# FurkanOM/tf-ssd

Measured on AMD Instinct MI355X. Metric: images/sec SSD300 (MobileNetV2) fwd+NMS, higher is better.
Workload: dtype f32

## Files before the change

include/ssd_hip.h:

```cpp
#ifndef SSD_HIP_H
#define SSD_HIP_H

#include <stddef.h>
#include <stdint.h>

#ifdef __cplusplus
extern "C" {
#endif

#define SSD_OK 0
#define SSD_E_INVALID (-1)
#define SSD_E_HIP (-2)
#define SSD_E_UNSUPPORTED (-3)
#define SSD_E_STATE (-4)

const char* ssd_version(void);
const char* ssd_last_error(void);
int ssd_init(int device);
void* ssd_stream_create(int high_priority);
void* ssd_stream_create_masked(const unsigned* cu_mask, int words);
int ssd_stream_destroy(void* stream);

int ssd_priors_count(const int* fmaps, const int* n_ars, int levels);
int ssd_priors(const int* fmaps, const float* const* ars, const int* n_ars, int levels,
// ... 337 lines not shown
#define SSD_LOC_HUBER 0
#define SSD_LOC_IOU 1
#define SSD_LOC_GIOU 2
#define SSD_LOC_DIOU 3
#define SSD_LOC_CIOU 4
int ssd_iou_loc_loss_tile(void);
size_t ssd_iou_loc_loss_workspace_bytes(int B, int N);
int ssd_iou_loc_loss(const float* priors_dev, const float* variances, const float* actual_deltas_dev,
                     const float* pred_deltas_dev, int B, int N, int mode, float loc_loss_alpha,
                     float* loc_loss_dev, float* per_anchor_out_dev, float* grad_deltas_dev, float grad_scale,
                     void* workspace_dev, size_t workspace_bytes, void* stream);

#define SSD_LOSS_HARD_NEGATIVE 0
#define SSD_LOSS_FOCAL 1
typedef struct ssd_loss_config {
    int kind;
    float neg_pos_ratio, loc_loss_alpha, focal_alpha, focal_gamma;
    int loc_kind;
    const float* priors_dev;
    float variances[4];
} ssd_loss_config;
size_t ssd_loss_config_bytes(void);


enum ssd_act { SSD_ACT_NONE = 0, SSD_ACT_RELU = 1, SSD_ACT_RELU6 = 2 };

typedef struct ssd_conv_desc {
    int B, H, W, Cin;
    int Cout, kh, kw;
    int stride, dilation;
    int pad_t, pad_l, pad_b, pad_r;
    int act;
    int has_residual;
} ssd_conv_desc;

int ssd_same_pads(int in, int k, int stride, int dilation, int* before, int* after);
int ssd_conv_out_size(int in, int k, int stride, int dilation, int pad_before, int pad_after);

size_t ssd_conv_packed_weight_floats(int kh, int kw, int Cin, int Cout);
int ssd_conv_pack_weights(const float* hwio_dev, int kh, int kw, int Cin, int Cout,
                          float* packed_dev, void* stream);

int ssd_conv2d(const ssd_conv_desc* d, const float* in_dev, const float* packed_w_dev,
               const float* scale_dev, const float* shift_dev, const float* residual_dev,
               float* out_dev, long out_batch_stride, long out_pixel_stride, void* stream);

int ssd_conv_num_configs(void);
const char* ssd_conv_config_name(int config);
int ssd_conv2d_ex(const ssd_conv_desc* d, const float* in_dev, const float* packed_w_dev,
                  const float* scale_dev, const float* shift_dev, const float* residual_dev,
                  float* out_dev, long out_batch_stride, long out_pixel_stride, int config,
                  int split_k, float* splitk_ws_dev, void* stream);

int ssd_split_planes(const float* x_dev, long n, int channels, int planes, void* planes_dev, long plane_stride, void* stream);
int ssd_join_planes(const void* planes_dev, long n, int channels, int planes, long plane_stride, float* x_dev, void* stream);
int ssd_conv2d_planes(const ssd_conv_desc* d, const void* in_planes_dev, int planes, long in_plane_stride,
                      const float* packed_w_dev, const float* scale_dev, const float* shift_dev,
                      const float* residual_dev, float* out_dev, long out_batch_stride, long out_pixel_stride,
                      void* out_planes_dev, long out_plane_stride, int config, int split_k,
                      float* splitk_ws_dev, void* stream);

size_t ssd_conv_f16x2_weight_bytes(int kh, int kw, int Cin, int Cout);
int ssd_conv_pack_weights_f16x2(const float* packed_w_dev, int kh, int kw, int Cin, int Cout, void* w_planes_dev,
                                int* k_out, void* stream);
int ssd_conv2d_planes_f16x2(const ssd_conv_desc* d, const void* in_planes_dev, long in_plane_stride,
                            const float* packed_w_dev, const void* w_planes_dev, int w_exp, const float* scale_dev,
// ... 139 lines not shown
```

tf-ssd_amd/csrc/ssd_conv.h:

```cpp
#pragma once
#include <cmath>
#include <cstring>

#include "common.h"

namespace ssd {

struct ConvParams {
    const float* in;
    const float* w;
    const short* w3;
    const float* scale;
    const float* shift;
    const float* residual;
    float* out;
    int B, H, W, Cin, Ho, Wo, Cout;
    int kh, kw, stride, dil, pad_t, pad_l;
    int K, Kpad, Npad;
    long M;
    long out_batch_stride, out_pixel_stride;
    int n_split;
    float* out2;
    long out2_batch_stride, out2_pixel_stride;
    int vec_store2;
    int act;
    int vec_store;
    int split_k;
    float* partial;
    const float* wino_w;
    int bf16;
    const short* xp;
    long xp_plane;
    int xp_np;
    short* op;
    long op_plane;
    int op_np;
    const short* wh;
    float acc_scale;
};
inline int conv_vec_store(const ConvParams& p) {
    return (((uintptr_t)p.out & 15) == 0) && (p.out_pixel_stride % 4 == 0) && (p.out_batch_stride % 4 == 0);
}

struct FusedBlockParams {
    const float* x;
    float* y;
    const float* we;
    const float *es, *eh;
    const float* wd;
    const float *ds, *dh;
    const float* wp;
    const float *ps, *ph;
    int residual;
    int B, H, W, Cin, Ce, Cout, Ho, Wo, stride, pad_t, pad_l;
    int kpad_e, kpad_p, npad_p;
    int tiles_y, tiles_x;
    int bf16;
    int groups;
    const short* we3;
    const short* wp3;
    int bands;
    float* slabs;
    unsigned* tickets;
    float* e_out;
    short* y_planes;
    long y_plane;
    short* e_planes;
    long e_plane;
    int planes_np;
    int e_planes_np;
    int planes_only;
// ... 168 lines not shown
```

tf-ssd_amd/csrc/ssd_conv.hip:

```cpp
#include <cstring>

#include "ssd_conv.h"
#include "ssd_conv_mfma.h"

namespace ssd {


template <int V>
__global__ void splitk_reduce_kernel(const ConvParams p) {
    const long total = p.M * p.Cout;
    const long groups = total / V;
    const int HoWo = p.Ho * p.Wo;
    for (long g = (long)blockIdx.x * blockDim.x + threadIdx.x; g < groups; g += (long)gridDim.x * blockDim.x) {
        float t[V];
#pragma unroll
        for (int j = 0; j < V; ++j) t[j] = 0.f;
        for (int s = 0; s < p.split_k; ++s) {
            const float* src = p.partial + (long)s * total + g * V;
            if (V == 4) {
                const f32x4 v = *reinterpret_cast<const f32x4*>(src);
#pragma unroll
                for (int j = 0; j < V; ++j) t[j] += v[j];
            } else {
                t[0] += src[0];
// ... 400 lines not shown
    return SSD_OK;
}

int launch_pack_weights(const float* hwio, int K, int Cout, int Kpad, int Npad, float* packed, hipStream_t st) {
    const long total = (long)Npad * Kpad;
    if (total == 0) return SSD_OK;
    const int blocks = (int)(cdiv(total, 256) < 4096 ? cdiv(total, 256) : 4096);
    hipLaunchKernelGGL(pack_weights_kernel, dim3(blocks), dim3(256), 0, st, hwio, K, Cout, Kpad, Npad, packed);
    SSD_LAUNCH_CHECK();
    return SSD_OK;
}

int fill_conv_params(const ssd_conv_desc* d, ConvParams* p) {
    SSD_CHECK_ARG(d != nullptr, "conv2d: descriptor is NULL");
    SSD_CHECK_ARG(d->B >= 0 && d->H >= 1 && d->W >= 1 && d->Cin >= 1 && d->Cout >= 1,
                  "conv2d: bad tensor sizes B=%d H=%d W=%d Cin=%d Cout=%d", d->B, d->H, d->W, d->Cin, d->Cout);
    SSD_CHECK_ARG(d->kh >= 1 && d->kw >= 1 && d->stride >= 1 && d->dilation >= 1,
                  "conv2d: bad kernel %dx%d stride %d dilation %d", d->kh, d->kw, d->stride, d->dilation);
    SSD_CHECK_ARG(d->pad_t >= 0 && d->pad_l >= 0 && d->pad_b >= 0 && d->pad_r >= 0, "conv2d: negative padding");
    SSD_CHECK_ARG(d->act >= 0 && d->act <= 2, "conv2d: unknown activation %d", d->act);
    const int Ho = ssd_conv_out_size(d->H, d->kh, d->stride, d->dilation, d->pad_t, d->pad_b);
    const int Wo = ssd_conv_out_size(d->W, d->kw, d->stride, d->dilation, d->pad_l, d->pad_r);
    SSD_CHECK_ARG(Ho >= 1 && Wo >= 1, "conv2d: empty output (%d x %d)", Ho, Wo);
    *p = ConvParams{};
    p->B = d->B; p->H = d->H; p->W = d->W; p->Cin = d->Cin; p->Ho = Ho; p->Wo = Wo; p->Cout = d->Cout;
    p->kh = d->kh; p->kw = d->kw; p->stride = d->stride; p->dil = d->dilation;
    p->pad_t = d->pad_t; p->pad_l = d->pad_l;
    p->K = d->kh * d->kw * d->Cin;
    p->Kpad = conv_kpad(p->K);
    p->Npad = conv_npad(d->Cout);
    p->M = (long)d->B * Ho * Wo;
    p->act = d->act;
    p->split_k = 1;
    return SSD_OK;
}

}

using namespace ssd;

static int bind_conv_io(ConvParams& p, const ssd_conv_desc* d, const char* who, const float* residual_dev, float* out_dev,
                        long out_batch_stride, long out_pixel_stride, int split_k, float* splitk_ws_dev) {
    SSD_CHECK_ARG(!d->has_residual || residual_dev, "%s: has_residual set but residual is NULL", who);
    p.residual = d->has_residual ? residual_dev : nullptr;
    p.out = out_dev;
    p.out_pixel_stride = out_pixel_stride > 0 ? out_pixel_stride : p.Cout;
    p.out_batch_stride = out_batch_stride > 0 ? out_batch_stride : (long)p.Ho * p.Wo * p.out_pixel_stride;
    p.vec_store = conv_vec_store(p);
    if (split_k > 1) {
        SSD_CHECK_ARG(splitk_ws_dev != nullptr, "%s: split_k > 1 needs a workspace", who);
        p.split_k = split_k;
        p.partial = splitk_ws_dev;
    }
    return SSD_OK;
}

extern "C" {

int ssd_same_pads(int in, int k, int stride, int dilation, int* before, int* after) {
    if (in < 1 || k < 1 || stride < 1 || dilation < 1) return SSD_E_INVALID;
    const int out = (in + stride - 1) / stride;
    const int keff = (k - 1) * dilation + 1;
    int p = (out - 1) * stride + keff - in;
    if (p < 0) p = 0;
    if (before) *before = p / 2;
    if (after) *after = p - p / 2;
// ... 186 lines not shown
```

tf-ssd_amd/csrc/ssd_convdma.hip:

```cpp
#include "ssd_block_common.h"
#include "ssd_conv_mfma.h"

namespace ssd {

template <int MT, int NT, int WM, int WN, int NP, bool GEMM1X1, int KSH = 1>
__device__ __forceinline__ void conv_dma_body(const ConvParams& p, char* __restrict__ dsm) {
    constexpr int KS = NP == 1 ? 2 : NP == 2 ? KSH : 1;
    constexpr int WPL = NP == 1 ? 3 : 0;
    constexpr int BM = 16 * MT * WM, BN = 16 * NT * WN, NW = WM * WN;
    constexpr int RBX = BM / 16, RBW = BN / 16;
    constexpr int RPX = (RBX + NW - 1) / NW, RPW = (RBW + NW - 1) / NW;
    constexpr int XBYTES = KS * NP * BM * 64, STAGE = KS * NP * (BM + BN) * 64;

    const int tid = threadIdx.x, lane = tid & 63;
    const int wave = __builtin_amdgcn_readfirstlane(tid >> 6);
    const int wm = wave / WN, wn = wave % WN;
    const int nb_n = (p.Cout + BN - 1) / BN;
    const int mblk = blockIdx.x / nb_n, nblk = blockIdx.x - mblk * nb_n;
    const long m0 = (long)mblk * BM;
    const int n0 = nblk * BN;
    const int HoWo = p.Ho * p.Wo;
    const int ntaps = p.kh * p.kw;

    const int r16 = lane >> 2;
    const int q8 = ((lane & 3) ^ ((lane >> 3) & 3)) * 8;
    const int b_first = (int)(m0 / HoWo);
    const long npix = (long)p.B * p.H * p.W;
    const long xbase_e = (GEMM1X1 ? m0 : (long)b_first * p.H * p.W) * 32;
    const long xrange = min((long)0x7fffffffL, (npix * p.Cin - xbase_e) * 2);
    const int slice_b = (int)(npix * 64);
    __amdgpu_buffer_rsrc_t xrs[NP];
#pragma unroll
    for (int pl = 0; pl < NP; ++pl)
        xrs[pl] = __builtin_amdgcn_make_buffer_rsrc(const_cast<short*>(p.xp + pl * p.xp_plane + xbase_e), 0, (int)xrange, 0x00020000);
    const long wplane_b = (long)p.Npad * p.Kpad * 2;
    const __amdgpu_buffer_rsrc_t wrs = __builtin_amdgcn_make_buffer_rsrc(const_cast<short*>(NP == 2 ? p.wh : p.w3), 0, (int)((NP == 2 ? 2 : 4) * wplane_b), 0x00020000);

    int xoff[RPX];
// ... 111 lines not shown
#pragma unroll
    for (int mi = 0; mi < MT; ++mi)
#pragma unroll
        for (int ni = 0; ni < NT; ++ni) acc[mi][ni] = f32x4{0.f, 0.f, 0.f, 0.f};

    const int frow = lane & 15;
    const int fq = ((lane >> 4) ^ ((frow >> 1) & 3)) << 4;
    auto mma_tile = [&](int stage, int ns) {
        const char* sb = dsm + stage * STAGE;
#pragma unroll
        for (int s = 0; s < KS; ++s) {
            if (KS > 1 && s >= ns) break;
            const char* Xb = sb + s * NP * BM * 64;
            const char* Wb = sb + XBYTES + s * NP * BN * 64;
            BP<NP> b[MT];
#pragma unroll
            for (int mi = 0; mi < MT; ++mi) {
                const char* r = Xb + ((wm * MT + mi) * 16 + frow) * 64 + fq;
#pragma unroll
                for (int pl = 0; pl < NP; ++pl) b[mi].p[pl] = *reinterpret_cast<const bf16x8*>(r + pl * BM * 64);
            }
#pragma unroll
            for (int ni = 0; ni < NT; ++ni) {
                const char* r = Wb + ((wn * NT + ni) * 16 + frow) * 64 + fq;
                BP<NP> a;
#pragma unroll
                for (int pl = 0; pl < NP; ++pl) a.p[pl] = *reinterpret_cast<const bf16x8*>(r + pl * BN * 64);
#pragma unroll
                for (int mi = 0; mi < MT; ++mi) acc[mi][ni] = mmaN<NP>(a, b[mi], acc[mi][ni]);
            }
        }
    };

    int ns_cur = 1;
    if (kt_begin < kt_end) {
        tile_setup(kt_begin);
        ns_cur = steps_here();
        issue(0);
    }
    asm volatile("s_waitcnt vmcnt(0)" ::: "memory");
    __syncthreads();
    for (int kt = kt_begin; kt < kt_end; ++kt) {
        const int stage = (kt - kt_begin) & 1;
        int ns_next = 1;
        if (kt + 1 < kt_end) {
            tile_advance();
            ns_next = steps_here();
            issue(stage ^ 1);
        }
        mma_tile(stage, ns_cur);
        ns_cur = ns_next;
        asm volatile("s_waitcnt vmcnt(0)" ::: "memory");
        __syncthreads();
    }
    if constexpr (NP == 2) {
#pragma unroll
        for (int mi = 0; mi < MT; ++mi)
#pragma unroll
            for (int ni = 0; ni < NT; ++ni) acc[mi][ni] *= p.acc_scale;
    }
    conv_epilogue<MT, NT>(p, acc, m0, n0, wm, wn, lane, HoWo);
}

template <int MT, int NT, int WM, int WN, int NP, bool GEMM1X1, int KSH = 1>
__global__ __launch_bounds__(64 * WM * WN) void conv_dma_kernel(const ConvParams p) {
    extern __shared__ __attribute__((aligned(1024))) char dsm_dma[];
    conv_dma_body<MT, NT, WM, WN, NP, GEMM1X1, KSH>(p, dsm_dma);
}

namespace {

typedef void (*convd_kernel_t)(const ConvParams);
struct ConvDCfg {
    const char* name3;
    const char* name1;
    const char* nameh;
    const char* nameh2;
    int BM, BN, threads;
    convd_kernel_t gemm3, general3, gemm1, general1, gemmh, generalh, gemmh2, generalh2;
};
template <int MT, int NT, int WM, int WN, bool GEMM1X1>
constexpr convd_kernel_t dmah_ks2_kernel() {
    if constexpr (16 * MT * WM + 16 * NT * WN <= 320) return conv_dma_kernel<MT, NT, WM, WN, 2, GEMM1X1, 2>;
    else return nullptr;
}
#define DCFG(MT, NT, WM, WN)                                                                                  \
    {"dma3_" #MT "x" #NT "_" #WM "x" #WN, "dmab_" #MT "x" #NT "_" #WM "x" #WN, "dmah_" #MT "x" #NT "_" #WM "x" #WN,          \
     "dmah_" #MT "x" #NT "_" #WM "x" #WN "_ks2", 16 * MT * WM, 16 * NT * WN, 64 * WM * WN,                       \
     conv_dma_kernel<MT, NT, WM, WN, 3, true>, conv_dma_kernel<MT, NT, WM, WN, 3, false>,                       \
     conv_dma_kernel<MT, NT, WM, WN, 1, true>, conv_dma_kernel<MT, NT, WM, WN, 1, false>,                       \
     conv_dma_kernel<MT, NT, WM, WN, 2, true>, conv_dma_kernel<MT, NT, WM, WN, 2, false>,                       \
     dmah_ks2_kernel<MT, NT, WM, WN, true>(), dmah_ks2_kernel<MT, NT, WM, WN, false>()}
const ConvDCfg kCfgD[] = {
    DCFG(4, 4, 4, 2),
    DCFG(2, 4, 4, 2),
    DCFG(4, 4, 2, 4),
    DCFG(4, 2, 4, 2),
    DCFG(2, 7, 8, 1),
    DCFG(4, 5, 4, 2),
    DCFG(4, 4, 2, 2),
    DCFG(2, 7, 4, 1),
    DCFG(2, 5, 2, 2),
    DCFG(2, 4, 6, 2),
    DCFG(3, 4, 4, 3),
    DCFG(2, 4, 8, 2),
    DCFG(2, 2, 2, 2),
    DCFG(2, 5, 6, 2),
};
constexpr int kNumCfgD = sizeof(kCfgD) / sizeof(kCfgD[0]);
struct DmahList {
    int n = 0, tile[2 * kNumCfgD], ks[2 * kNumCfgD];
    DmahList() {
        for (int i = 0; i < kNumCfgD; ++i) { tile[n] = i; ks[n++] = 1; }
        for (int i = 0; i < kNumCfgD; ++i)
            if (kCfgD[i].gemmh2) { tile[n] = i; ks[n++] = 2; }
    }
};
const DmahList& dmah_list() {
    static const DmahList l;
    return l;
}

__global__ __launch_bounds__(256) void split_planes_kernel(const float* __restrict__ x, const long n4, const int C, const int np,
                                                           short* __restrict__ planes, const long plane) {
    const long P = n4 * 4 / C;
// ... 30 lines not shown
    for (long e = (long)blockIdx.x * 256 + threadIdx.x; e < total; e += (long)gridDim.x * 256) {
        const long n = e / Kpad;
        const long d = Npad ? plane_elem(n, (int)(e - n * Kpad), Npad) : e;
        unsigned h, l;
        split_h2(w[e] * scale, 0.f, h, l);
        out[d] = (short)(h & 0xffffu);
        out[total + d] = (short)(l & 0xffffu);
    }
}

int dma_num_configs() { return kNumCfgD; }
const char* dma3_config_name(int i) { return kCfgD[i].name3; }
const char* dmab_config_name(int i) { return kCfgD[i].name1; }
bool dma_config_valid(int i, int np, const ConvParams& p) {
    const short* wpl = np == 2 ? p.wh : p.w3;
    if (!p.xp || !wpl || p.xp_np != np) return false;
    if (((uintptr_t)p.xp & 15) || ((uintptr_t)wpl & 15) || (p.xp_plane & 7)) return false;
    if (p.M > 0x7fffffffL - 1024) return false;
    if (4 * (long)p.Npad * p.Kpad * 2 > 0x7fffffffL) return false;
    if ((long)p.B * p.H * p.W * p.Cin * 2 > 0x7fffffffL) return false;
    if (conv_is_gemm1x1(p)) return p.Cin % 32 == 0;
    if (p.kh * p.kw > 32) return false;
    if (((long)kCfgD[i].BM / (p.Ho * p.Wo) + 3) * p.H * p.W * 64 > 0x3fffffffL) return false;
    return p.Cin % (np == 1 ? 64 : 32) == 0;
}
bool dma3_config_valid(int i, const ConvParams& p) { return dma_config_valid(i, 3, p); }
bool dmab_config_valid(int i, const ConvParams& p) { return dma_config_valid(i, 1, p); }
long dma_grid_blocks(int i, const ConvParams& p) {
    return ((p.M + kCfgD[i].BM - 1) / kCfgD[i].BM) * ((p.Cout + kCfgD[i].BN - 1) / kCfgD[i].BN);
}
int dma3_k_tiles(int, const ConvParams& p) { return (p.K + 31) / 32; }
int dmab_k_tiles(int, const ConvParams& p) { return (p.K + 31) / 32 / 2; }

int dma_launch(const ConvParams& p, int i, convd_kernel_t gemm, convd_kernel_t general, int stage_planes, hipStream_t st) {
    const long blocks = dma_grid_blocks(i, p);
    SSD_UNSUPPORTED_IF(blocks > 0x7fffffffL, "conv2d: grid too large");
    const ConvDCfg& g = kCfgD[i];
    const convd_kernel_t fn = conv_is_gemm1x1(p) ? gemm : general;
    const int lds = 2 * stage_planes * (g.BM + g.BN) * 64;
    if (lds > 64 * 1024) SSD_HIP(hipFuncSetAttribute(reinterpret_cast<const void*>(fn), hipFuncAttributeMaxDynamicSharedMemorySize, lds));
    dim3 grid((unsigned)blocks, p.split_k > 1 ? p.split_k : 1);
    hipLaunchKernelGGL(fn, grid, dim3(g.threads), lds, st, p);
    SSD_LAUNCH_CHECK();
    return SSD_OK;
}
int dma3_launch(const ConvParams& p, int i, hipStream_t st) { return dma_launch(p, i, kCfgD[i].gemm3, kCfgD[i].general3, 3, st); }
int dmab_launch(const ConvParams& p, int i, hipStream_t st) { return dma_launch(p, i, kCfgD[i].gemm1, kCfgD[i].general1, 2, st); }

int dmah_num_configs() { return dmah_list().n; }
const char* dmah_config_name(int j) {
    const DmahList& l = dmah_list();
    return l.ks[j] == 2 ? kCfgD[l.tile[j]].nameh2 : kCfgD[l.tile[j]].nameh;
}
bool dmah_config_valid(int j, const ConvParams& p) {
    if (!(p.acc_scale > 0.f)) return false;
    return dma_config_valid(dmah_list().tile[j], 2, p);
}
long dmah_grid_blocks(int j, const ConvParams& p) { return dma_grid_blocks(dmah_list().tile[j], p); }
int dmah_k_tiles(int j, const ConvParams& p) {
    const int ks = dmah_list().ks[j];
    if (conv_is_gemm1x1(p)) return ((p.K + 31) / 32 + ks - 1) / ks;
    return p.kh * p.kw * ((p.Cin / 32 + ks - 1) / ks);
}
int dmah_launch(const ConvParams& p, int j, hipStream_t st) {
    const ConvDCfg& g = kCfgD[dmah_list().tile[j]];
    if (dmah_list().ks[j] == 2) return dma_launch(p, dmah_list().tile[j], g.gemmh2, g.generalh2, 4, st);
    return dma_launch(p, dmah_list().tile[j], g.gemmh, g.generalh, 2, st);
}

}

#ifndef __HIP_DEVICE_COMPILE__
const ConvFamily kConvDma3 = {CF_DMA3, dma_num_configs, dma3_config_name, dma3_config_valid, dma_grid_blocks, dma3_k_tiles, dma3_launch,
                              CONV_READS_PLANES | CONV_NET_FP32 | CONV_WRITES_PLANES | CONV_SPLITK_REDUCE};
const ConvFamily kConvDmab = {CF_DMAB, dma_num_configs, dmab_config_name, dmab_config_valid, dma_grid_blocks, dmab_k_tiles, dmab_launch,
                              CONV_READS_PLANES | CONV_NET_BF16 | CONV_WRITES_PLANES | CONV_SPLITK_REDUCE};
const ConvFamily kConvDmah = {CF_DMAH, dmah_num_configs, dmah_config_name, dmah_config_valid, dmah_grid_blocks, dmah_k_tiles, dmah_launch,
                              CONV_READS_F16X2 | CONV_NET_FP32 | CONV_WRITES_PLANES | CONV_SPLITK_REDUCE};
#endif
int dmah_tile_index(int j) { return dmah_list().tile[j]; }

int launch_absmax_bits(const float* packed, int K, int Cout, unsigned* absmax_bits_dev, hipStream_t st) {
    const long total = (long)conv_kpad(K) * conv_npad(Cout);
    if (total == 0) return SSD_OK;
    const int blocks = (int)((total + 255) / 256 < 1024 ? (total + 255) / 256 : 1024);
    hipLaunchKernelGGL(absmax_bits_kernel, dim3(blocks), dim3(256), 0, st, packed, total, absmax_bits_dev);
    SSD_LAUNCH_CHECK();
    return SSD_OK;
}
int launch_pack_f16x2(const float* packed, int K, int Cout, int k, short* planes, hipStream_t st, bool row_major) {
    const long total = (long)conv_kpad(K) * conv_npad(Cout);
    if (total == 0) return SSD_OK;
    const int blocks = (int)((total + 255) / 256 < 8192 ? (total + 255) / 256 : 8192);
    hipLaunchKernelGGL(pack_f16x2_kernel, dim3(blocks), dim3(256), 0, st, packed, total, conv_kpad(K), row_major ? 0 : conv_npad(Cout), ldexpf(1.f, k), planes);
    SSD_LAUNCH_CHECK();
    return SSD_OK;
}

int launch_split_planes(const float* x, long n, int C, int np, short* planes, long plane, hipStream_t st) {
// ... 23 lines not shown
```

tf-ssd_amd/csrc/ssd_net.h:

```cpp
#pragma once
#include <map>
#include <set>
#include <string>
#include <vector>

#include "ssd_conv.h"

struct ssd_train_state;
void ssd_train_state_free(ssd_train_state*);

namespace ssd {

enum LayerKind { LK_CONV = 0, LK_DW, LK_POOL, LK_L2NORM, LK_SOFTMAX, LK_FUSED };
static const char* kKindName[] = {"conv", "dw", "pool", "l2norm", "softmax", "fused"};

enum Route { RT_OFF = 0, RT_LAYER, RT_STEM, RT_DWPROJ, RT_TILE, RT_BAND, RT_BAND3, RT_IMAGE, RT_IMAGE_SPLIT };
inline bool route_is_image(Route r) { return r == RT_IMAGE || r == RT_IMAGE_SPLIT; }

struct Param {
    std::string name;
    std::vector<int> shape;
    size_t count = 0;
    float* dev = nullptr;
    bool set = false;
// ... 97 lines not shown
    int wait[2] = {-1, -1};
    bool after_main = false;
    bool publishes = false;
    bool join_first = false;
};

}

struct ssd_net {
    int backbone = 0, img_size = 300, levels = 6, L = 21;
    std::vector<int> n_ars;
    std::vector<ssd::Param> params;
    std::map<std::string, int> param_index;
    std::vector<ssd::Tensor> tensors;
    std::map<std::string, int> tensor_index;
    std::vector<ssd::Layer> layers;
    std::vector<int> fmap;
    std::vector<long> level_off;
    int num_priors = 0;
    bool finalized = false;
    bool fuse_blocks = true;
    bool fuse_softmax = true;
    bool fuse_dwproj = true;
    bool use_wino = true;
    int precision = 0;
    int fuse_band = 2;
    int fuse_image = 1;
    int lanes_hint = 1;
    bool tail_on_side = false;
    bool image_split = true;
    bool image_v2 = true;
    bool conv_dma = true;
    bool conv_f16x2 = true;
    bool image_f16x2 = true;
    bool plane_only = true;
    bool image_ticket = false;
    float* img_slabs = nullptr;
    unsigned* img_tickets = nullptr;
    int max_batch = 0;
    int last_batch = 0;
    std::vector<float*> owned;
    float* arena = nullptr;
    size_t arena_bytes = 0, plane_bytes = 0, slab_bytes = 0;
    size_t wplane_bytes = 0;
    size_t iplane_bytes = 0;
    float* splitk_ws = nullptr;
    size_t splitk_floats = 0;
    float* deltas = nullptr;
    float* probs = nullptr;
    void* nms_ws = nullptr;
    size_t nms_ws_bytes = 0;
    int nms_ws_batch = 0;
    int nms_ws_total = 0;
    int scratch_batch = 0;
    std::map<std::string, std::pair<std::string, int>> preset;
    int n_preset = 0;
    int n_autotuned = 0;
    bool launch_raced = false;
    bool use_graph = true;
    bool graphs_unsafe = false;
    bool use_graph_auto = true;
    struct GraphEntry {
        std::vector<const void*> key;
        hipGraphExec_t exec = nullptr;
        hipGraph_t graph = nullptr;
        const float* image = nullptr;
// ... 68 lines not shown
```

tf-ssd_amd/csrc/ssd_net.hip:

```cpp
#include <algorithm>
#include <cstdlib>
#include <cstring>
#include <map>
#include <memory>
#include <string>
#include <vector>

#include "ssd_net.h"

using namespace ssd;

namespace ssd {

struct Builder {
    ssd_net& net;
    explicit Builder(ssd_net& n) : net(n) {}

    int add_param(const std::string& name, std::vector<int> shape) {
        Param p;
        p.name = name;
        p.shape = std::move(shape);
        p.count = 1;
        for (int d : p.shape) p.count *= (size_t)d;
        net.params.push_back(p);
// ... 235 lines not shown
    const int conv8_2 = x;
    x = b.conv("conv9_1", "conv9_1", x, 128, 1, 1, 0, 1, "", true, SSD_ACT_RELU);
    x = b.conv("conv9_2", "conv9_2", x, 256, 3, 2, 1, 1, "", true, SSD_ACT_RELU);
    const int conv9_2 = x;
    x = b.conv("conv10_1", "conv10_1", x, 128, 1, 1, 0, 1, "", true, SSD_ACT_RELU);
    x = b.conv("conv10_2", "conv10_2", x, 256, 3, 1, 0, 1, "", true, SSD_ACT_RELU);
    const int conv10_2 = x;
    x = b.conv("conv11_1", "conv11_1", x, 128, 1, 1, 0, 1, "", true, SSD_ACT_RELU);
    x = b.conv("conv11_2", "conv11_2", x, 256, 3, 1, 0, 1, "", true, SSD_ACT_RELU);
    const int conv11_2 = x;
    Layer l;
    l.name = "l2_normalization";
    l.kind = LK_L2NORM;
    l.in = conv4_3;
    const Tensor t = net.tensors[conv4_3];
    l.H = l.Ho = t.H; l.W = l.Wo = t.W; l.Cin = l.Cout = t.C;
    l.p_gamma = b.add_param("l2_normalization/scale", {t.C});
    l.out = b.add_tensor("l2_normalization", t.H, t.W, t.C);
    net.layers.push_back(l);
    b.heads({l.out, conv7, conv8_2, conv9_2, conv10_2, conv11_2});
}

ConvParams layer_conv_params(const ssd_net& net, const Layer& l, int B, const float* in, float* out, const float* res,
                             float* deltas_out, float* probs_out) {
    ConvParams p{};
    p.in = in;
    p.w = l.packed;
    p.w3 = conv_split_planes(l.packed, l.kh * l.kw * l.Cin, l.Cout);
    p.bf16 = net.precision;
    if (l.wh) {
        p.wh = reinterpret_cast<const short*>(l.wh);
        p.acc_scale = ldexpf(1.f, -(8 + l.wh_k));
    }
    if (l.in >= 0 && net.tensors[l.in].planes) {
        const Tensor& ti = net.tensors[l.in];
        p.xp = ti.planes; p.xp_plane = ti.plane_stride; p.xp_np = ti.planes_np;
    }
    if (l.out >= 0 && l.head_kind == 0 && net.tensors[l.out].planes_live && (l.Cout & 3) == 0) {
        const Tensor& to = net.tensors[l.out];
        p.op = to.planes; p.op_plane = to.plane_stride; p.op_np = to.planes_np;
    }
    p.wino_w = l.wino;
    p.scale = l.scale;
    p.shift = l.shift;
    p.residual = res;
    p.B = B; p.H = l.H; p.W = l.W; p.Cin = l.Cin; p.Ho = l.Ho; p.Wo = l.Wo; p.Cout = l.Cout;
    p.kh = l.kh; p.kw = l.kw; p.stride = l.stride; p.dil = l.dil; p.pad_t = l.pt; p.pad_l = l.pl;
    p.K = l.kh * l.kw * l.Cin;
    p.Kpad = conv_kpad(p.K);
    p.Npad = conv_npad(l.Cout);
    p.M = (long)B * l.Ho * l.Wo;
    p.act = l.act;
    p.split_k = l.split_k;
    p.partial = l.splitk_part ? l.splitk_part : net.splitk_ws;
    if (l.head_kind == 0) {
        p.out = l.out >= 0 && net.tensors[l.out].plane_only && p.op ? nullptr : out;
        p.out_pixel_stride = l.Cout;
        p.out_batch_stride = (long)l.Ho * l.Wo * l.Cout;
    } else {
        conv_route_head(p, l, probs_out, deltas_out);
    }
    p.vec_store = conv_vec_store(p);
    return p;
}

static FusedBlockParams fused_shape(const ssd_net& net, const Layer& f, int B) {
// ... 1033 lines not shown
}

int ssd_net_predict_cfg(ssd_net* net, const float* image_dev, int B, const float* priors_dev, const float* var,
                        const ssd_nms_config* cfg, float* boxes_dev, float* labels_dev, float* scores_dev,
                        int* valid_dev, void* stream) {
    SSD_CHECK_ARG(cfg != nullptr, "ssd_net_predict_cfg: config is NULL");
    return predict_impl(net, image_dev, B, priors_dev, var, cfg->max_total, cfg->iou_threshold, cfg->score_threshold, cfg,
                        boxes_dev, labels_dev, scores_dev, valid_dev, stream);
}

struct OptionSpec {
    const char* name;
    bool ssd_net::*flag;
    int ssd_net::*num;
    int lo, hi, refinalize;
};
static const OptionSpec kOptions[] = {
    {"fuse_blocks", &ssd_net::fuse_blocks, nullptr, 0, 1, 0},
    {"precision", nullptr, &ssd_net::precision, 0, 1, 1},
    {"fuse_band", nullptr, &ssd_net::fuse_band, 0, 2, 0},
    {"fuse_image", nullptr, &ssd_net::fuse_image, 0, 2, 0},
    {"lanes_hint", nullptr, &ssd_net::lanes_hint, 1, 8, 0},
    {"tail_on_side", &ssd_net::tail_on_side, nullptr, 0, 1, 0},
    {"image_split", &ssd_net::image_split, nullptr, 0, 1, 1},
    {"image_ticket", &ssd_net::image_ticket, nullptr, 0, 1, 0},
    {"fuse_softmax", &ssd_net::fuse_softmax, nullptr, 0, 1, 0},
    {"fuse_dwproj", &ssd_net::fuse_dwproj, nullptr, 0, 1, 0},
    {"overlap_heads", &ssd_net::overlap_heads, nullptr, 0, 1, 0},
    {"use_wino", &ssd_net::use_wino, nullptr, 0, 1, 2},
    {"image_v2", &ssd_net::image_v2, nullptr, 0, 1, 0},
    {"conv_dma", &ssd_net::conv_dma, nullptr, 0, 1, 1},
    {"conv_f16x2", &ssd_net::conv_f16x2, nullptr, 0, 1, 1},
    {"image_f16x2", &ssd_net::image_f16x2, nullptr, 0, 1, 1},
    {"plane_only", &ssd_net::plane_only, nullptr, 0, 1, 0},
    {"use_graph", &ssd_net::use_graph, nullptr, 0, 1, 0},
};

int ssd_net_set_option(ssd_net* net, const char* name, int value) {
    SSD_CHECK_ARG(net && name, "ssd_net_set_option: NULL argument");
    const std::string n(name);
    const OptionSpec* o = nullptr;
    for (const OptionSpec& k : kOptions)
        if (n == k.name) o = &k;
    if (!o) {
        set_error("ssd_net_set_option: unknown option '%s'", name);
        return SSD_E_INVALID;
    }
    if (n == "precision") SSD_CHECK_ARG(value == 0 || value == 1, "ssd_net_set_option: precision must be 0 (fp32) or 1 (bf16)");
    if (n == "use_graph") {
        if (value && net->graphs_unsafe && net->overlap_heads) {
            set_error("ssd_net_set_option: use_graph 1 needs overlap_heads 0 with GPU_MAX_HW_QUEUES < 4 (hipGraph capture of the forked step crashes in the runtime; a single in-order stream replays fine)");
            return SSD_E_UNSUPPORTED;
        }
        net->use_graph_auto = false;
    }
    const int v = o->flag ? value != 0 : std::min(std::max(value, o->lo), o->hi);
    const int old = o->flag ? (int)(net->*o->flag) : net->*o->num;
    if (o->flag) net->*o->flag = v != 0;
    else net->*o->num = v;
    if (o->refinalize == 2 || (o->refinalize == 1 && v != old)) net->finalized = false;
    net->drop_graphs();
    resolve_routes(*net);
    if (n == "fuse_softmax" && net->nms_ws) {
        (void)hipDeviceSynchronize();
        SSD_HIP(hipMemset(net->nms_ws, 0, net->nms_ws_bytes));
    }
// ... 180 lines not shown
```

tf-ssd_amd/ssd_hip.py:

```python
import ctypes
import os
import sys


def configure_serving(lanes=3):
    if "GPU_MAX_HW_QUEUES" in os.environ:
        return os.environ["GPU_MAX_HW_QUEUES"] == str(lanes)
    t = sys.modules.get("torch")
    try:
        if t is not None and t.cuda.is_initialized():
            return False
    except Exception:
        return False
    os.environ["GPU_MAX_HW_QUEUES"] = str(int(lanes))
    return True


if os.environ.get("SSD_HIP_HW_QUEUES", "").isdigit() and int(os.environ["SSD_HIP_HW_QUEUES"]) > 0:
    configure_serving(int(os.environ["SSD_HIP_HW_QUEUES"]))

import numpy as np
import torch

_HERE = os.path.dirname(os.path.abspath(__file__))
LIB_PATH = os.environ.get("SSD_HIP_LIBRARY") or os.path.join(_HERE, "libssd_hip.so")

c_float_p = ctypes.POINTER(ctypes.c_float)
c_int_p = ctypes.POINTER(ctypes.c_int)
vp = ctypes.c_void_p


class ConvDesc(ctypes.Structure):
    _fields_ = [(n, ctypes.c_int) for n in (
        "B", "H", "W", "Cin", "Cout", "kh", "kw", "stride", "dilation",
        "pad_t", "pad_l", "pad_b", "pad_r", "act", "has_residual")]


class ResizeDesc(ctypes.Structure):
    _fields_ = [("src_offset", ctypes.c_longlong), ("tmp_offset", ctypes.c_longlong)] + [(n, ctypes.c_int) for n in (
        "H", "W", "h_bounds", "h_k", "h_ksize", "v_bounds", "v_k", "v_ksize")]


class JpegInfo(ctypes.Structure):
    _fields_ = [("width", ctypes.c_int), ("height", ctypes.c_int), ("components", ctypes.c_int),
                ("h_samp", ctypes.c_int * 3), ("v_samp", ctypes.c_int * 3), ("quant_index", ctypes.c_int * 3),
                ("restart_interval", ctypes.c_int), ("mcus_x", ctypes.c_int), ("mcus_y", ctypes.c_int),
                ("blocks_w", ctypes.c_int * 3), ("blocks_h", ctypes.c_int * 3), ("reserved", ctypes.c_int),
                ("coef_offset", ctypes.c_longlong * 3), ("coef_bytes", ctypes.c_longlong),
                ("quant", (ctypes.c_ushort * 64) * 3)]


class JpegHuff(ctypes.Structure):
    _fields_ = [("look", ctypes.c_ushort * 256), ("maxcode", ctypes.c_int * 17), ("valoff", ctypes.c_int * 17),
                ("vals", ctypes.c_ubyte * 256), ("reserved", ctypes.c_ubyte * 8)]


class JpegScanPlan(ctypes.Structure):
    _fields_ = [("data_begin", ctypes.c_longlong), ("data_end", ctypes.c_longlong), ("segments", ctypes.c_int),
                ("reserved", ctypes.c_int), ("huff", JpegHuff * 6)]


class PngInfo(ctypes.Structure):
    _fields_ = [(n, ctypes.c_int) for n in ("width", "height", "depth", "color_type", "channels", "filter_distance",
                                            "palette_entries", "idat_count")] + [
        (n, ctypes.c_longlong) for n in ("row_bytes", "stream_bytes", "idat_bytes", "first_idat")] + [
        ("palette", ctypes.c_ubyte * 768)]


# ... 437 lines not shown
```

Measured before the change: 68230.

## Add three-stage LDS ring pipeline for fp16-pair DMA conv kernels

Adds a three-stage ring buffer variant of the buffer-load-to-LDS conv kernel for the fp16-pair path. The next tile's loads are interleaved with the MFMA loop, and the wait uses partial vmcnt counts so a prefetch stays in flight across the barrier. The aim is to hide global-to-LDS latency better than the two-stage scheme, which waits for all loads to finish before each barrier. It costs 1.5x the LDS per block, which may reduce occupancy. The ring is on by default through the dma_ring option and falls back to two stages when the tile does not fit.

```diff
diff --git a/include/ssd_hip.h b/include/ssd_hip.h
--- a/include/ssd_hip.h
+++ b/include/ssd_hip.h
@@ -393,6 +393,7 @@
     int pad_t, pad_l, pad_b, pad_r;
     int act;
     int has_residual;
+    int dma_two_stage;
 } ssd_conv_desc;
 
 int ssd_same_pads(int in, int k, int stride, int dilation, int* before, int* after);
diff --git a/tf-ssd_amd/csrc/ssd_conv.h b/tf-ssd_amd/csrc/ssd_conv.h
--- a/tf-ssd_amd/csrc/ssd_conv.h
+++ b/tf-ssd_amd/csrc/ssd_conv.h
@@ -37,6 +37,7 @@
     int op_np;
     const short* wh;
     float acc_scale;
+    int dma_two_stage;
 };
 inline int conv_vec_store(const ConvParams& p) {
     return (((uintptr_t)p.out & 15) == 0) && (p.out_pixel_stride % 4 == 0) && (p.out_batch_stride % 4 == 0);
diff --git a/tf-ssd_amd/csrc/ssd_conv.hip b/tf-ssd_amd/csrc/ssd_conv.hip
--- a/tf-ssd_amd/csrc/ssd_conv.hip
+++ b/tf-ssd_amd/csrc/ssd_conv.hip
@@ -456,6 +456,7 @@
     p->M = (long)d->B * Ho * Wo;
     p->act = d->act;
     p->split_k = 1;
+    p->dma_two_stage = d->dma_two_stage != 0;
     return SSD_OK;
 }
 
diff --git a/tf-ssd_amd/csrc/ssd_convdma.hip b/tf-ssd_amd/csrc/ssd_convdma.hip
--- a/tf-ssd_amd/csrc/ssd_convdma.hip
+++ b/tf-ssd_amd/csrc/ssd_convdma.hip
@@ -1,9 +1,11 @@
+#include <type_traits>
+
 #include "ssd_block_common.h"
 #include "ssd_conv_mfma.h"
 
 namespace ssd {
 
-template <int MT, int NT, int WM, int WN, int NP, bool GEMM1X1, int KSH = 1>
+template <int MT, int NT, int WM, int WN, int NP, bool GEMM1X1, int KSH = 1, int NST = 2>
 __device__ __forceinline__ void conv_dma_body(const ConvParams& p, char* __restrict__ dsm) {
     constexpr int KS = NP == 1 ? 2 : NP == 2 ? KSH : 1;
     constexpr int WPL = NP == 1 ? 3 : 0;
@@ -181,26 +183,107 @@
         }
     };
 
-    int ns_cur = 1;
-    if (kt_begin < kt_end) {
-        tile_setup(kt_begin);
-        ns_cur = steps_here();
-        issue(0);
-    }
-    asm volatile("s_waitcnt vmcnt(0)" ::: "memory");
-    __syncthreads();
-    for (int kt = kt_begin; kt < kt_end; ++kt) {
-        const int stage = (kt - kt_begin) & 1;
-        int ns_next = 1;
-        if (kt + 1 < kt_end) {
+    if constexpr (NST == 3) {
+        static_assert(NP == 2 && KS == 1, "the ring is the one-k-step fp16-pair loop");
+        static_assert(3 * STAGE <= 160 * 1024, "three stages of this tile do not fit the LDS");
+        constexpr int NPX = RPX * NP, NPC = (RPX + RPW) * NP;
+        const int skipped = (RBX % NW != 0 && wave + (RPX - 1) * NW >= RBX ? NP : 0) + (RBW % NW != 0 && wave + (RPW - 1) * NW >= RBW ? NP : 0);
+        auto piece = [&](char* sb, int q) {
+            if (q < NPX) {
+                const int j = q / NP, pl = q % NP, rb = wave + j * NW;
+                if (RBX % NW != 0 && rb >= RBX) return;
+                const bool ok = GEMM1X1 ? (xvalid[j] != 0) : (((xvalid[j] >> l_tap) & 1u) != 0);
+                const int vo = ok ? xoff[j] + l_xtile : (int)0x80000000;
+                __builtin_amdgcn_raw_ptr_buffer_load_lds(xrs[pl], (lds_dst_t)(sb + (pl * BM + rb * 16) * 64), 16, vo, l_xs, 0, 0);
+            } else {
+                const int j = (q - NPX) / NP, pl = (q - NPX) % NP, rb = wave + j * NW;
+                if (RBW % NW != 0 && rb >= RBW) return;
+                __builtin_amdgcn_raw_ptr_buffer_load_lds(wrs, (lds_dst_t)(sb + XBYTES + (pl * BN + rb * 16) * 64), 16, woff[j],
+                                                         (int)(pl * wplane_b) + (l_k0 >> 5) * p.Npad * 64, 0, 0);
+            }
+        };
+        auto wait_newest = [&]() {
+            if (skipped == 0) asm volatile("s_waitcnt vmcnt(%0)" ::"n"(NPC) : "memory");
+            else if (skipped == NP) asm volatile("s_waitcnt vmcnt(%0)" ::"n"(NPC - NP) : "memory");
+            else asm volatile("s_waitcnt vmcnt(%0)" ::"n"(NPC - 2 * NP) : "memory");
+        };
+        auto ring_tile = [&](const char* rd, char* wr, auto copy) {
+            const char* Wb = rd + XBYTES;
+            BP<NP> b[MT], a, an;
+#pragma unroll
+            for (int mi = 0; mi < MT; ++mi) {
+                const char* r = rd + ((wm * MT + mi) * 16 + frow) * 64 + fq;
+#pragma unroll
+                for (int pl = 0; pl < NP; ++pl) b[mi].p[pl] = *reinterpret_cast<const bf16x8*>(r + pl * BM * 64);
+            }
+#pragma unroll
+            for (int pl = 0; pl < NP; ++pl) a.p[pl] = *reinterpret_cast<const bf16x8*>(Wb + (wn * NT * 16 + frow) * 64 + fq + pl * BN * 64);
+#pragma unroll
+            for (int ni = 0; ni < NT; ++ni) {
+                if (ni + 1 < NT) {
+#pragma unroll
+                    for (int pl = 0; pl < NP; ++pl) an.p[pl] = *reinterpret_cast<const bf16x8*>(Wb + ((wn * NT + ni + 1) * 16 + frow) * 64 + fq + pl * BN * 64);
+                }
+#pragma unroll
+                for (int mi = 0; mi < MT; ++mi) acc[mi][ni] = mmaN<NP>(a, b[mi], acc[mi][ni]);
+                if constexpr (decltype(copy)::value) {
+#pragma unroll
+                    for (int q = ni * NPC / NT; q < (ni + 1) * NPC / NT; ++q) piece(wr, q);
+                }
+                a = an;
+            }
+        };
+        const int nt = max(kt_end - kt_begin, 0);
+        if (nt > 0) {
+            tile_setup(kt_begin);
+#pragma unroll
+            for (int q = 0; q < NPC; ++q) piece(dsm, q);
+        }
+        if (nt > 1) {
             tile_advance();
-            ns_next = steps_here();
-            issue(stage ^ 1);
-        }
-        mma_tile(stage, ns_cur);
-        ns_cur = ns_next;
+#pragma unroll
+            for (int q = 0; q < NPC; ++q) piece(dsm + STAGE, q);
+            wait_newest();
+        } else {
+            asm volatile("s_waitcnt vmcnt(0)" ::: "memory");
+        }
+        lds_barrier();
+        int st = 0, i = 0;
+        for (; i + 2 < nt; ++i) {
+            tile_advance();
+            ring_tile(dsm + st * STAGE, dsm + (st == 0 ? 2 : st - 1) * STAGE, std::true_type{});
+            wait_newest();
+            lds_barrier();
+            st = st == 2 ? 0 : st + 1;
+        }
+        for (; i < nt; ++i) {
+            ring_tile(dsm + st * STAGE, nullptr, std::false_type{});
+            asm volatile("s_waitcnt vmcnt(0)" ::: "memory");
+            lds_barrier();
+            st = st == 2 ? 0 : st + 1;
+        }
+    } else {
+        int ns_cur = 1;
+        if (kt_begin < kt_end) {
+            tile_setup(kt_begin);
+            ns_cur = steps_here();
+            issue(0);
+        }
         asm volatile("s_waitcnt vmcnt(0)" ::: "memory");
         __syncthreads();
+        for (int kt = kt_begin; kt < kt_end; ++kt) {
+            const int stage = (kt - kt_begin) & 1;
+            int ns_next = 1;
+            if (kt + 1 < kt_end) {
+                tile_advance();
+                ns_next = steps_here();
+                issue(stage ^ 1);
+            }
+            mma_tile(stage, ns_cur);
+            ns_cur = ns_next;
+            asm volatile("s_waitcnt vmcnt(0)" ::: "memory");
+            __syncthreads();
+        }
     }
     if constexpr (NP == 2) {
 #pragma unroll
@@ -211,10 +294,10 @@
     conv_epilogue<MT, NT>(p, acc, m0, n0, wm, wn, lane, HoWo);
 }
 
-template <int MT, int NT, int WM, int WN, int NP, bool GEMM1X1, int KSH = 1>
+template <int MT, int NT, int WM, int WN, int NP, bool GEMM1X1, int KSH = 1, int NST = 2>
 __global__ __launch_bounds__(64 * WM * WN) void conv_dma_kernel(const ConvParams p) {
     extern __shared__ __attribute__((aligned(1024))) char dsm_dma[];
-    conv_dma_body<MT, NT, WM, WN, NP, GEMM1X1, KSH>(p, dsm_dma);
+    conv_dma_body<MT, NT, WM, WN, NP, GEMM1X1, KSH, NST>(p, dsm_dma);
 }
 
 namespace {
@@ -227,7 +310,14 @@
     const char* nameh2;
     int BM, BN, threads;
     convd_kernel_t gemm3, general3, gemm1, general1, gemmh, generalh, gemmh2, generalh2;
+    convd_kernel_t gemmhr, generalhr;
 };
+constexpr int dmah_stages(int BM, int BN) { return 3 * 2 * (BM + BN) * 64 <= 160 * 1024 ? 3 : 2; }
+template <int MT, int NT, int WM, int WN, bool GEMM1X1>
+constexpr convd_kernel_t dmah_ring_kernel() {
+    if constexpr (dmah_stages(16 * MT * WM, 16 * NT * WN) == 3) return conv_dma_kernel<MT, NT, WM, WN, 2, GEMM1X1, 1, 3>;
+    else return nullptr;
+}
 template <int MT, int NT, int WM, int WN, bool GEMM1X1>
 constexpr convd_kernel_t dmah_ks2_kernel() {
     if constexpr (16 * MT * WM + 16 * NT * WN <= 320) return conv_dma_kernel<MT, NT, WM, WN, 2, GEMM1X1, 2>;
@@ -239,7 +329,8 @@
      conv_dma_kernel<MT, NT, WM, WN, 3, true>, conv_dma_kernel<MT, NT, WM, WN, 3, false>,                       \
      conv_dma_kernel<MT, NT, WM, WN, 1, true>, conv_dma_kernel<MT, NT, WM, WN, 1, false>,                       \
      conv_dma_kernel<MT, NT, WM, WN, 2, true>, conv_dma_kernel<MT, NT, WM, WN, 2, false>,                       \
-     dmah_ks2_kernel<MT, NT, WM, WN, true>(), dmah_ks2_kernel<MT, NT, WM, WN, false>()}
+     dmah_ks2_kernel<MT, NT, WM, WN, true>(), dmah_ks2_kernel<MT, NT, WM, WN, false>(),                         \
+     dmah_ring_kernel<MT, NT, WM, WN, true>(), dmah_ring_kernel<MT, NT, WM, WN, false>()}
 const ConvDCfg kCfgD[] = {
     DCFG(4, 4, 4, 2),
     DCFG(2, 4, 4, 2),
@@ -336,12 +427,12 @@
 int dma3_k_tiles(int, const ConvParams& p) { return (p.K + 31) / 32; }
 int dmab_k_tiles(int, const ConvParams& p) { return (p.K + 31) / 32 / 2; }
 
-int dma_launch(const ConvParams& p, int i, convd_kernel_t gemm, convd_kernel_t general, int stage_planes, hipStream_t st) {
+int dma_launch(const ConvParams& p, int i, convd_kernel_t gemm, convd_kernel_t general, int stage_planes, hipStream_t st, int stages = 2) {
     const long blocks = dma_grid_blocks(i, p);
     SSD_UNSUPPORTED_IF(blocks > 0x7fffffffL, "conv2d: grid too large");
     const ConvDCfg& g = kCfgD[i];
     const convd_kernel_t fn = conv_is_gemm1x1(p) ? gemm : general;
-    const int lds = 2 * stage_planes * (g.BM + g.BN) * 64;
+    const int lds = stages * stage_planes * (g.BM + g.BN) * 64;
     if (lds > 64 * 1024) SSD_HIP(hipFuncSetAttribute(reinterpret_cast<const void*>(fn), hipFuncAttributeMaxDynamicSharedMemorySize, lds));
     dim3 grid((unsigned)blocks, p.split_k > 1 ? p.split_k : 1);
     hipLaunchKernelGGL(fn, grid, dim3(g.threads), lds, st, p);
@@ -369,6 +460,7 @@
 int dmah_launch(const ConvParams& p, int j, hipStream_t st) {
     const ConvDCfg& g = kCfgD[dmah_list().tile[j]];
     if (dmah_list().ks[j] == 2) return dma_launch(p, dmah_list().tile[j], g.gemmh2, g.generalh2, 4, st);
+    if (!p.dma_two_stage && g.gemmhr) return dma_launch(p, dmah_list().tile[j], g.gemmhr, g.generalhr, 2, st, 3);
     return dma_launch(p, dmah_list().tile[j], g.gemmh, g.generalh, 2, st);
 }
 
diff --git a/tf-ssd_amd/csrc/ssd_net.h b/tf-ssd_amd/csrc/ssd_net.h
--- a/tf-ssd_amd/csrc/ssd_net.h
+++ b/tf-ssd_amd/csrc/ssd_net.h
@@ -153,6 +153,7 @@
     bool image_v2 = true;
     bool conv_dma = true;
     bool conv_f16x2 = true;
+    bool dma_ring = true;
     bool image_f16x2 = true;
     bool plane_only = true;
     bool image_ticket = false;
diff --git a/tf-ssd_amd/csrc/ssd_net.hip b/tf-ssd_amd/csrc/ssd_net.hip
--- a/tf-ssd_amd/csrc/ssd_net.hip
+++ b/tf-ssd_amd/csrc/ssd_net.hip
@@ -291,6 +291,7 @@
         p.wh = reinterpret_cast<const short*>(l.wh);
         p.acc_scale = ldexpf(1.f, -(8 + l.wh_k));
     }
+    p.dma_two_stage = !net.dma_ring;
     if (l.in >= 0 && net.tensors[l.in].planes) {
         const Tensor& ti = net.tensors[l.in];
         p.xp = ti.planes; p.xp_plane = ti.plane_stride; p.xp_np = ti.planes_np;
@@ -1390,6 +1391,7 @@
     {"conv_dma", &ssd_net::conv_dma, nullptr, 0, 1, 1},
     {"conv_f16x2", &ssd_net::conv_f16x2, nullptr, 0, 1, 1},
     {"image_f16x2", &ssd_net::image_f16x2, nullptr, 0, 1, 1},
+    {"dma_ring", &ssd_net::dma_ring, nullptr, 0, 1, 0},
     {"plane_only", &ssd_net::plane_only, nullptr, 0, 1, 0},
     {"use_graph", &ssd_net::use_graph, nullptr, 0, 1, 0},
 };
diff --git a/tf-ssd_amd/ssd_hip.py b/tf-ssd_amd/ssd_hip.py
--- a/tf-ssd_amd/ssd_hip.py
+++ b/tf-ssd_amd/ssd_hip.py
@@ -33,7 +33,7 @@
 class ConvDesc(ctypes.Structure):
     _fields_ = [(n, ctypes.c_int) for n in (
         "B", "H", "W", "Cin", "Cout", "kh", "kw", "stride", "dilation",
-        "pad_t", "pad_l", "pad_b", "pad_r", "act", "has_residual")]
+        "pad_t", "pad_l", "pad_b", "pad_r", "act", "has_residual", "dma_two_stage")]
 
 
 class ResizeDesc(ctypes.Structure):
```

After: 69430 (median of 6 runs). 1.8% higher.
